# Ipuch/cocofest

Hardware: AMD Instinct MI355X
Metric: NLP callback evals/s (constraint+Jac) and wall-clock to Ipopt-equiv convergence (higher is better)
Workload: dtype f64; 1 GPU; cfg2: OcpFes DingModelFrequency n_stim=10 @10Hz, final_time=1s, n_shooting=20, end_node_tracking=100N, RK1 x 10 multiple shooting; one step = g + J_g of every instance; batch_per_gpu=1048576, nv=42, ng=40, nnz_jac=100, parallelism=instances sharded over 1 GPU(s), no data-path collective

## Files before the change

### cocofest_amd/csrc/cfx_chain.hip

```cpp
#include <hip/hip_runtime.h>

#include <algorithm>
#include <string>

#include "../../include/cfx.h"
#include "cfx_inertia.h"
#include "cfx_internal.h"

namespace cfx_chain {

typedef double d4 __attribute__((ext_vector_type(4)));

struct Chain {
    double *D, *L, *U;
    double *Cl, *Cr;
    int64_t stride, wstride;
    int M;
};

template <int SP>
__device__ __forceinline__ double* cur_u(const Chain& C, int64_t b, int k, int h) {
    constexpr int64_t NB = (int64_t)SP * SP;
    return h == 1 ? C.U + b * C.stride + k * NB : C.Cl + b * C.wstride + (k + h / 2) * NB;
}
template <int SP>
__device__ __forceinline__ double* cur_l(const Chain& C, int64_t b, int k, int h) {
    constexpr int64_t NB = (int64_t)SP * SP;
    return h == 1 ? C.L + b * C.stride + k * NB : C.Cr + b * C.wstride + (k - h / 2) * NB;
}

template <int SP, class AF>
__device__ __forceinline__ d4 tile_mm(const AF& a_at, const double (&breg)[SP / 4], int I, d4 acc) {
    const int lane = threadIdx.x & 63;
    const int r = 16 * I + (lane & 15), kq = lane >> 4;
#pragma unroll
    for (int kk = 0; kk < SP / 4; ++kk) acc = __builtin_amdgcn_mfma_f64_16x16x4f64(a_at(r, 4 * kk + kq), breg[kk], acc, 0, 0, 0);
    return acc;
}

template <int SP>
__device__ __forceinline__ void load_bcol(const double* __restrict__ B, int J, double (&breg)[SP / 4]) {
    const int lane = threadIdx.x & 63;
#pragma unroll
    for (int kk = 0; kk < SP / 4; ++kk) breg[kk] = B[(4 * kk + (lane >> 4)) * SP + 16 * J + (lane & 15)];
}

template <int SP>
__device__ __forceinline__ void store_tile(double* __restrict__ C, int I, int J, d4 v) {
    const int lane = threadIdx.x & 63;
#pragma unroll
    for (int r = 0; r < 4; ++r) C[(16 * I + (lane >> 4) + 4 * r) * SP + 16 * J + (lane & 15)] = v[r];
}

__device__ __forceinline__ double pivot_key(double v, int r) {
    const uint64_t bits = (uint64_t)__double_as_longlong(fabs(v));
    if (bits >= 0x7ff0000000000000ull) return -1.0;
    return __longlong_as_double((long long)((bits & ~0x7Full) | (uint64_t)(127 - r)));
}

#define CFX_DPP_MAX(v, CTRL, RM, BM)                                                                              \
    do {                                                                                                          \
        const int lo_ = __double2loint(v), hi_ = __double2hiint(v);                                               \
        const int slo_ = __builtin_amdgcn_update_dpp(lo_, lo_, CTRL, RM, BM, false);                              \
        const int shi_ = __builtin_amdgcn_update_dpp(hi_, hi_, CTRL, RM, BM, false);                              \
        v = fmax(v, __hiloint2double(shi_, slo_));                                                                \
    } while (0)
__device__ __forceinline__ double wave_max(double v) {
    CFX_DPP_MAX(v, 0x111, 0xf, 0xf);
    CFX_DPP_MAX(v, 0x112, 0xf, 0xf);
    CFX_DPP_MAX(v, 0x114, 0xf, 0xf);
    CFX_DPP_MAX(v, 0x118, 0xf, 0xf);
    CFX_DPP_MAX(v, 0x142, 0xa, 0xf);
    CFX_DPP_MAX(v, 0x143, 0xc, 0xf);
    const int lo = __builtin_amdgcn_readlane(__double2loint(v), 63), hi = __builtin_amdgcn_readlane(__double2hiint(v), 63);
    return __hiloint2double(hi, lo);
}

constexpr int kNT = 256;

__device__ __forceinline__ double readlane_d(double v, int l) {
    return __hiloint2double(__builtin_amdgcn_readlane(__double2hiint(v), l), __builtin_amdgcn_readlane(__double2loint(v), l));
}

template <int SP>
__global__ void __launch_bounds__(kNT) k_chain_elim(Chain C, int first, int step, int h, int32_t* __restrict__ info) {
    constexpr int T = SP / 16;
    static_assert(SP % 16 == 0 && SP <= 128 && kNT == 256, "16-column panels; 7-bit row index in the pivot key");
    constexpr int LDA = SP + 1;
    __shared__ double A[SP * LDA];
    __shared__ uint8_t prow[SP], pstep[SP];
    const int t = threadIdx.x, lane = t & 63, wave = t >> 6;
    const int i = first + step * blockIdx.x;
    const int64_t b = blockIdx.y;
    if (i >= C.M) return;
    constexpr int64_t NB = (int64_t)SP * SP;
    double* D = C.D + b * C.stride + i * NB;
    for (int e = t; e < SP * SP; e += kNT) A[(e / SP) * LDA + e % SP] = D[e];
    for (int r = t; r < SP; r += kNT) pstep[r] = 255;
    __syncthreads();
    int sing = 0;
    bool used0 = false, used1 = false;
    const bool has0 = lane < SP, has1 = lane + 64 < SP;
#pragma unroll 1
    for (int j = 0; j < T; ++j) {
        if (wave == 0) {
            double a0[16], a1[16];
#pragma unroll
            for (int c = 0; c < 16; ++c) {
                a0[c] = has0 ? A[lane * LDA + 16 * j + c] : 0.0;
                a1[c] = has1 ? A[(lane + 64) * LDA + 16 * j + c] : 0.0;
            }
#pragma unroll
            for (int kk = 0; kk < 16; ++kk) {
                const int k = 16 * j + kk;
                double key = -1.0;
                if (has0 && !used0) key = pivot_key(a0[kk], lane);
                if (has1 && !used1) key = fmax(key, pivot_key(a1[kk], lane + 64));
                key = wave_max(key);
                int p;
                if (key >= 0.0) {
                    p = 127 - (int)((uint64_t)__double_as_longlong(key) & 0x7Full);
                } else {
                    const unsigned long long m0 = __ballot(has0 && !used0), m1 = __ballot(has1 && !used1);
                    p = m0 ? __ffsll((long long)m0) - 1 : 64 + __ffsll((long long)m1) - 1;
                    if (!sing) sing = k + 1;
                }
                used0 = used0 || p == lane;
                used1 = used1 || p == lane + 64;
                if (lane == 0) prow[k] = (uint8_t)p, pstep[p] = (uint8_t)k;
                double prv[16];
                if (p < 64) {
#pragma unroll
                    for (int c = 0; c < 16; ++c) prv[c] = readlane_d(a0[c], p);
                } else {
#pragma unroll
                    for (int c = 0; c < 16; ++c) prv[c] = readlane_d(a1[c], p - 64);
                }
                const double pv = prv[kk];
                if (pv == 0.0 && !sing) sing = k + 1;
                const double inv = pv != 0.0 ? 1.0 / pv : 0.0;
                double sc[16];
#pragma unroll
                for (int c = 0; c < 16; ++c) sc[c] = c == kk ? inv : prv[c] * inv;
                const bool ip0 = lane == p, ip1 = lane + 64 == p;
                const double m0 = a0[kk], m1 = a1[kk];
#pragma unroll
                for (int c = 0; c < 16; ++c) {
                    if (c == kk) continue;
                    a0[c] = ip0 ? sc[c] : fma(-m0, sc[c], a0[c]);
                    a1[c] = ip1 ? sc[c] : fma(-m1, sc[c], a1[c]);
                }
                a0[kk] = ip0 ? inv : -m0 * inv;
                a1[kk] = ip1 ? inv : -m1 * inv;
            }
#pragma unroll
            for (int c = 0; c < 16; ++c) {
                if (has0) A[lane * LDA + 16 * j + c] = a0[c];
                if (has1) A[(lane + 64) * LDA + 16 * j + c] = a1[c];
            }
        }
        __syncthreads();
        for (int q = wave; q < T - 1; q += kNT / 64) {
            const int Jc = q < j ? q : q + 1;
            double breg[4];
#pragma unroll
            for (int kk = 0; kk < 4; ++kk) breg[kk] = A[prow[16 * j + 4 * kk + (lane >> 4)] * LDA + 16 * Jc + (lane & 15)];
#pragma unroll 1
            for (int I = 0; I < T; ++I) {
                d4 acc;
#pragma unroll
                for (int r = 0; r < 4; ++r) {
                    const int row = 16 * I + (lane >> 4) + 4 * r;
                    const int ps = pstep[row];
                    const bool piv = ps >= 16 * j && ps < 16 * j + 16;
                    acc[r] = piv ? 0.0 : A[row * LDA + 16 * Jc + (lane & 15)];
                }
#pragma unroll
                for (int kk = 0; kk < 4; ++kk)
                    acc = __builtin_amdgcn_mfma_f64_16x16x4f64(A[(16 * I + (lane & 15)) * LDA + 16 * j + 4 * kk + (lane >> 4)],
                                                               breg[kk], acc, 0, 0, 0);
#pragma unroll
                for (int r = 0; r < 4; ++r) A[(16 * I + (lane >> 4) + 4 * r) * LDA + 16 * Jc + (lane & 15)] = acc[r];
            }
        }
        __syncthreads();
    }
    const int tr = t >> 4, tc = t & 15;
    double a[T][T];
#pragma unroll
    for (int ii = 0; ii < T; ++ii)
#pragma unroll
        for (int jj = 0; jj < T; ++jj) a[ii][jj] = A[prow[tr + 16 * ii] * LDA + pstep[tc + 16 * jj]];
    __syncthreads();
#pragma unroll
    for (int ii = 0; ii < T; ++ii)
#pragma unroll
        for (int jj = 0; jj < T; ++jj) A[(tr + 16 * ii) * LDA + tc + 16 * jj] = a[ii][jj];
    __syncthreads();
    if (t == 0 && sing && info && info[b] == 0) info[b] = (int32_t)(i * SP + sing);
    for (int e = t; e < SP * SP; e += kNT) D[e] = A[(e / SP) * LDA + e % SP];
    auto a_at = [&](int r, int c) { return A[r * LDA + c]; };
    const bool xl = i - h >= 0, yu = i + h < C.M;
    for (int it = wave; it < 2 * (SP / 16); it += kNT / 64) {
        const int side = it / (SP / 16), J = it % (SP / 16);
        if (side == 0 ? !xl : !yu) continue;
        double* Bm = side == 0 ? cur_l<SP>(C, b, i, h) : cur_u<SP>(C, b, i, h);
        double breg[SP / 4];
        load_bcol<SP>(Bm, J, breg);
#pragma unroll 1
        for (int I = 0; I < SP / 16; ++I) {
            d4 acc = {0.0, 0.0, 0.0, 0.0};
            acc = tile_mm<SP>(a_at, breg, I, acc);
            store_tile<SP>(Bm, I, J, acc);
        }
    }
}

constexpr int kUpdGlobalB = 256;
template <int SP>
constexpr bool chain_b_fits() {
    return 2 * SP * (SP + 1) * 8 <= 150 * 1024;
}
template <int SP, bool BLDS>
constexpr size_t chain_upd_lds() {
    return (size_t)(BLDS ? 2 : 1) * SP * (SP + 1) * sizeof(double);
}
template <int SP, bool BLDS>
__global__ void __launch_bounds__(kNT) k_chain_upd(Chain C, int h) {
    constexpr int T16 = SP / 16, NT = T16 * T16, TPW = (NT + 3) / 4;
    constexpr int LD = SP + 1;
    constexpr bool BL = BLDS && chain_b_fits<SP>();
    extern __shared__ double sm[];
    double* sA = sm;
    double* sB = sm + SP * LD;
    const int t = threadIdx.x, wave = t >> 6, lane = t & 63;
    const int p = 2 * h * blockIdx.x, part = blockIdx.z;
    const int64_t b = blockIdx.y;
    if (p >= C.M) return;
    constexpr int64_t NB = (int64_t)SP * SP;
    const int i = p + h, j = p - h;
    const bool hi = i < C.M, hj = j >= 0;
    const bool hyi = hi && i + h < C.M;
    if ((part == 0 && !hi && !hj) || (part == 1 && !hi) || (part == 2 && !hj)) return;
    const double* Up = hi ? cur_u<SP>(C, b, p, h) : nullptr;
    const double* Lp = hj ? cur_l<SP>(C, b, p, h) : nullptr;
    d4 acc[TPW];
#pragma unroll
    for (int q = 0; q < TPW; ++q) acc[q] = d4{0.0, 0.0, 0.0, 0.0};
    auto product = [&](const double* __restrict__ Ag, const double* __restrict__ Bg) {
        __syncthreads();
        for (int e = t; e < SP * SP; e += kNT) {
            const int r = e / SP, c = e - r * SP;
            sA[r * LD + c] = Ag[e];
            if constexpr (BL) sB[r * LD + c] = Bg[e];
        }
        __syncthreads();
#pragma unroll
        for (int q = 0; q < TPW; ++q) {
            const int tile = wave + 4 * q;
            if (tile < NT) {
                const int I = tile / T16, J = tile % T16;
                const int ra = 16 * I + (lane & 15), kq = lane >> 4, cb = 16 * J + (lane & 15);
                d4 a = acc[q];
#pragma unroll
                for (int kk = 0; kk < SP / 4; ++kk) {
                    const double bv = BL ? sB[(4 * kk + kq) * LD + cb] : Bg[(4 * kk + kq) * SP + cb];
                    a = __builtin_amdgcn_mfma_f64_16x16x4f64(sA[ra * LD + 4 * kk + kq], bv, a, 0, 0, 0);
                }
                acc[q] = a;
            }
        }
    };
    double* out;
    if (part == 0) {
        if (hi) product(Up, cur_l<SP>(C, b, i, h));
        if (hj) product(Lp, cur_u<SP>(C, b, j, h));
        out = C.D + b * C.stride + p * NB;
    } else if (part == 1) {
        if (hyi) product(Up, cur_u<SP>(C, b, i, h));
        out = C.Cl + b * C.wstride + i * NB;
    } else {
        product(Lp, cur_l<SP>(C, b, j, h));
        out = C.Cr + b * C.wstride + j * NB;
    }
#pragma unroll
    for (int q = 0; q < TPW; ++q) {
        const int tile = wave + 4 * q;
        if (tile < NT) {
            const int I = tile / T16, J = tile % T16;
#pragma unroll
            for (int r = 0; r < 4; ++r) {
                const int64_t e = (16 * I + (lane >> 4) + 4 * r) * SP + 16 * J + (lane & 15);
                if (part == 0) out[e] -= acc[q][r];
                else out[e] = -acc[q][r];
            }
        }
    }
}

template <int SP>
__device__ __forceinline__ double row_dot(const double* __restrict__ Mx, int r, const double* x) {
    double a0 = 0.0, a1 = 0.0, a2 = 0.0, a3 = 0.0;
    const double* row = Mx + (int64_t)r * SP;
#pragma unroll 4
    for (int k = 0; k < SP; k += 4) {
        a0 = fma(row[k], x[k], a0);
        a1 = fma(row[k + 1], x[k + 1], a1);
        a2 = fma(row[k + 2], x[k + 2], a2);
        a3 = fma(row[k + 3], x[k + 3], a3);
    }
    return (a0 + a1) + (a2 + a3);
}

struct Rhs {
    double* R;
    int64_t r_inst, r_rhs;
    double* T;
    int64_t t_inst, t_rhs;
};

template <int SP>
__global__ void __launch_bounds__(kNT) k_chain_fwd(Chain C, Rhs X, int h) {
    static_assert(SP <= 128, "rows over two thread halves");
    __shared__ double vi[SP], vj[SP], ti[SP], tj[SP];
    const int t = threadIdx.x;
    const int p = 2 * h * blockIdx.x;
    const int64_t b = blockIdx.z, c = blockIdx.y;
    if (p >= C.M) return;
    constexpr int64_t NB = (int64_t)SP * SP;
    const int i = p + h, j = p - h;
    const bool hi = i < C.M, hj = j >= 0;
    double* R = X.R + b * X.r_inst + c * X.r_rhs;
    double* T = X.T + b * X.t_inst + c * X.t_rhs;
    for (int r = t; r < SP; r += kNT) {
        vi[r] = hi ? R[(int64_t)i * SP + r] : 0.0;
        vj[r] = hj ? R[(int64_t)j * SP + r] : 0.0;
    }
    __syncthreads();
    if (t < SP) {
        if (hi) {
            const double v = row_dot<SP>(C.D + b * C.stride + i * NB, t, vi);
            ti[t] = v;
            T[(int64_t)i * SP + t] = v;
        }
    } else if (t >= 128 && t < 128 + SP) {
        if (hj) tj[t - 128] = row_dot<SP>(C.D + b * C.stride + j * NB, t - 128, vj);
    }
    __syncthreads();
    if (t < SP) {
        if (hi) vi[t] = row_dot<SP>(cur_u<SP>(C, b, p, h), t, ti);
    } else if (t >= 128 && t < 128 + SP) {
        if (hj) vj[t - 128] = row_dot<SP>(cur_l<SP>(C, b, p, h), t - 128, tj);
    }
    __syncthreads();
    if (t < SP && (hi || hj)) {
        double acc = R[(int64_t)p * SP + t];
        if (hi) acc -= vi[t];
        if (hj) acc -= vj[t];
        R[(int64_t)p * SP + t] = acc;
    }
}

template <int SP>
__global__ void __launch_bounds__(kNT) k_chain_top(Chain C, Rhs X) {
    __shared__ double v[SP];
    const int t = threadIdx.x;
    const int64_t b = blockIdx.z, c = blockIdx.y;
    double* R = X.R + b * X.r_inst + c * X.r_rhs;
    for (int r = t; r < SP; r += kNT) v[r] = R[r];
    __syncthreads();
    if (t < SP) R[t] = row_dot<SP>(C.D + b * C.stride, t, v);
}

template <int SP>
__global__ void __launch_bounds__(kNT) k_chain_bwd(Chain C, Rhs X, int h) {
    __shared__ double xl[SP], xr[SP];
    const int t = threadIdx.x;
    const int i = h + 2 * h * blockIdx.x;
    const int64_t b = blockIdx.z, c = blockIdx.y;
    if (i >= C.M) return;
    const bool hr = i + h < C.M;
    double* R = X.R + b * X.r_inst + c * X.r_rhs;
    const double* T = X.T + b * X.t_inst + c * X.t_rhs;
    for (int r = t; r < SP; r += kNT) {
        xl[r] = R[(int64_t)(i - h) * SP + r];
        xr[r] = hr ? R[(int64_t)(i + h) * SP + r] : 0.0;
    }
    __syncthreads();
    __shared__ double yl[SP], yr[SP];
    if (t < SP) yl[t] = row_dot<SP>(cur_l<SP>(C, b, i, h), t, xl);
    else if (t >= 128 && t < 128 + SP && hr) yr[t - 128] = row_dot<SP>(cur_u<SP>(C, b, i, h), t - 128, xr);
    __syncthreads();
    if (t < SP) {
        double acc = T[(int64_t)i * SP + t] - yl[t];
        if (hr) acc -= yr[t];
        R[(int64_t)i * SP + t] = acc;
    }
}

static int levels(int M) {
    int L = 0;
    while ((1 << L) < M) ++L;
    return L;
}

template <int SP, bool BL>
static hipError_t allow_upd_lds() {
    if (chain_upd_lds<SP, BL>() <= 65536) return hipSuccess;
    static const hipError_t e = hipFuncSetAttribute(reinterpret_cast<const void*>(&k_chain_upd<SP, BL>),
                                                    hipFuncAttributeMaxDynamicSharedMemorySize,
                                                    (int)chain_upd_lds<SP, BL>());
    return e;
}

template <int SP>
static hipError_t factor_sp(const Chain& C, int64_t B, int32_t* info, hipStream_t s) {
    const int L = levels(C.M);
    constexpr bool FITS = chain_b_fits<SP>();
    hipError_t e = allow_upd_lds<SP, FITS>();
    if (e == hipSuccess) e = allow_upd_lds<SP, false>();
    if (e != hipSuccess) return e;
    for (int l = 0; l < L; ++l) {
        const int h = 1 << l;
        const int ne = (C.M - h + 2 * h - 1) / (2 * h), ns = (C.M + 2 * h - 1) / (2 * h);
        hipLaunchKernelGGL(k_chain_elim<SP>, dim3((unsigned)ne, (unsigned)B), dim3(kNT), 0, s, C, h, 2 * h, h, info);
        if (FITS && ns < kUpdGlobalB)
            k_chain_upd<SP, FITS><<<dim3((unsigned)ns, (unsigned)B, 3), dim3(kNT), chain_upd_lds<SP, FITS>(), s>>>(C, h);
        else
            k_chain_upd<SP, false><<<dim3((unsigned)ns, (unsigned)B, 3), dim3(kNT), chain_upd_lds<SP, false>(), s>>>(C, h);
    }
    hipLaunchKernelGGL(k_chain_elim<SP>, dim3(1, (unsigned)B), dim3(kNT), 0, s, C, 0, 1, 1 << L, info);
    return hipGetLastError();
}

template <int SP>
static hipError_t solve_sp(const Chain& C, int64_t B, const Rhs& X, int nrhs, hipStream_t s) {
    const int L = levels(C.M);
    for (int l = 0; l < L; ++l) {
        const int h = 1 << l;
        const int ns = (C.M + 2 * h - 1) / (2 * h);
        hipLaunchKernelGGL(k_chain_fwd<SP>, dim3((unsigned)ns, (unsigned)nrhs, (unsigned)B), dim3(kNT), 0, s, C, X, h);
    }
    hipLaunchKernelGGL(k_chain_top<SP>, dim3(1, (unsigned)nrhs, (unsigned)B), dim3(kNT), 0, s, C, X);
    for (int l = L - 1; l >= 0; --l) {
        const int h = 1 << l;
        const int ne = (C.M - h + 2 * h - 1) / (2 * h);
        hipLaunchKernelGGL(k_chain_bwd<SP>, dim3((unsigned)ne, (unsigned)nrhs, (unsigned)B), dim3(kNT), 0, s, C, X, h);
    }
    return hipGetLastError();
}

template <int SP>
constexpr size_t chain_inertia_lds() {
    return (size_t)SP * (SP + 1) * sizeof(double);
}
template <int SP>
__global__ void __launch_bounds__(kNT) k_chain_inertia(Chain C, int32_t* __restrict__ neg) {
    extern __shared__ double A[];
    constexpr int64_t NB = (int64_t)SP * SP;
    const int64_t b = blockIdx.y;
    const double* D = C.D + b * C.stride + blockIdx.x * NB;
    for (int e = threadIdx.x; e < SP * SP; e += kNT) {
        const int r = e / SP, c = e % SP;
        A[r * (SP + 1) + c] = 0.5 * (D[r * SP + c] + D[c * SP + r]);
    }
    __syncthreads();
    const int cnt = cfx_inertia::sym_neg_count(A, SP + 1, SP);
    if (threadIdx.x == 0 && cnt) atomicAdd(neg + b, cnt);
}

template <int SP>
static hipError_t inertia_sp(const Chain& C, int64_t B, int32_t* neg, hipStream_t s) {
    if (chain_inertia_lds<SP>() > 65536) {
        static const hipError_t e = hipFuncSetAttribute(reinterpret_cast<const void*>(&k_chain_inertia<SP>),
                                                        hipFuncAttributeMaxDynamicSharedMemorySize,
                                                        (int)chain_inertia_lds<SP>());
        if (e != hipSuccess) return e;
    }
    k_chain_inertia<SP><<<dim3((unsigned)C.M, (unsigned)B), dim3(kNT), chain_inertia_lds<SP>(), s>>>(C, neg);
    return hipGetLastError();
}

#define CFX_CHAIN_SP(F, ...)                                     \
    switch (sp) {                                                \
        case 16: e = F<16>(__VA_ARGS__); break;                  \
        case 32: e = F<32>(__VA_ARGS__); break;                  \
        case 48: e = F<48>(__VA_ARGS__); break;                  \
        case 64: e = F<64>(__VA_ARGS__); break;                  \
        case 80: e = F<80>(__VA_ARGS__); break;                  \
        case 96: e = F<96>(__VA_ARGS__); break;                  \
        case 112: e = F<112>(__VA_ARGS__); break;                \
        case 128: e = F<128>(__VA_ARGS__); break;                \
        default: e = hipErrorInvalidValue; break;                \
    }

}

int cfx_chain_sp_ok(int32_t sp) { return sp >= 16 && sp <= 128 && sp % 16 == 0; }

int cfx_chain_factor_s(int64_t batch, int32_t M, int32_t sp, double* D, double* L, double* U, int64_t stride,
                       double* Cl, double* Cr, int64_t wstride, int32_t* info, void* stream) {
    if (batch < 1 || batch > 65535 || M < 1 || !cfx_chain_sp_ok(sp) || !D || !L || !U || !Cl || !Cr) {
        g_create_error = "cfx_chain_factor: invalid argument";
        return CFX_EINVAL;
    }
    const hipStream_t s = (hipStream_t)stream;
    if (info && hipMemsetAsync(info, 0, batch * sizeof(int32_t), s) != hipSuccess) {
        g_create_error = "cfx_chain_factor: hipMemsetAsync failed";
        return CFX_EHIP;
    }
    const cfx_chain::Chain C{D, L, U, Cl, Cr, stride, wstride, M};
    hipError_t e;
    CFX_CHAIN_SP(cfx_chain::factor_sp, C, batch, info, s)
    if (e != hipSuccess) {
        g_create_error = std::string("cfx_chain_factor: ") + hipGetErrorString(e);
        return CFX_EHIP;
    }
    return CFX_OK;
}

int cfx_chain_solve_s(int64_t batch, int32_t M, int32_t sp, const double* D, const double* L, const double* U,
                      int64_t stride, const double* Cl, const double* Cr, int64_t wstride, int32_t nrhs, double* R,
                      int64_t r_inst, int64_t r_rhs, double* T, int64_t t_inst, int64_t t_rhs, void* stream) {
    if (batch < 1 || batch > 65535 || M < 1 || !cfx_chain_sp_ok(sp) || nrhs < 1 || nrhs > 65535 || !R || !T) {
        g_create_error = "cfx_chain_solve: invalid argument";
        return CFX_EINVAL;
    }
    const cfx_chain::Chain C{const_cast<double*>(D), const_cast<double*>(L), const_cast<double*>(U),
                             const_cast<double*>(Cl), const_cast<double*>(Cr), stride, wstride, M};
    const cfx_chain::Rhs X{R, r_inst, r_rhs, T, t_inst, t_rhs};
    hipError_t e;
    CFX_CHAIN_SP(cfx_chain::solve_sp, C, batch, X, nrhs, (hipStream_t)stream)
    if (e != hipSuccess) {
        g_create_error = std::string("cfx_chain_solve: ") + hipGetErrorString(e);
        return CFX_EHIP;
    }
    return CFX_OK;
}

int cfx_chain_inertia_s(int64_t batch, int32_t M, int32_t sp, const double* D, int64_t stride, int32_t* neg,
                        void* stream) {
    if (batch < 1 || batch > 65535 || M < 1 || !cfx_chain_sp_ok(sp) || !D || !neg) {
        g_create_error = "cfx_chain_inertia: invalid argument";
        return CFX_EINVAL;
    }
    const cfx_chain::Chain C{const_cast<double*>(D), nullptr, nullptr, nullptr, nullptr, stride, 0, M};
    hipError_t e;
    CFX_CHAIN_SP(cfx_chain::inertia_sp, C, batch, neg, (hipStream_t)stream)
    if (e != hipSuccess) {
        g_create_error = std::string("cfx_chain_inertia: ") + hipGetErrorString(e);
        return CFX_EHIP;
    }
    return CFX_OK;
}

extern "C" int cfx_btri_factor(int64_t batch, int32_t M, int32_t sp, double* D, double* L, double* U, double* work,
                               int32_t* info, void* stream) {
    if (!work) {
        g_create_error = "cfx_btri_factor: work is NULL";
        return CFX_EINVAL;
    }
    const int64_t st = (int64_t)M * sp * sp;
    return cfx_chain_factor_s(batch, M, sp, D, L, U, st, work, work + batch * st, st, info, stream);
}

extern "C" int cfx_btri_solve(int64_t batch, int32_t M, int32_t sp, const double* D, const double* L, const double* U,
                              const double* work, int32_t nrhs, double* rhs, double* scratch, void* stream) {
    if (!work) {
        g_create_error = "cfx_btri_solve: work is NULL";
        return CFX_EINVAL;
    }
    const int64_t st = (int64_t)M * sp * sp, nv = (int64_t)M * sp;
    return cfx_chain_solve_s(batch, M, sp, D, L, U, st, work, work + batch * st, st, nrhs, rhs, nrhs * nv, nv, scratch,
                             nrhs * nv, nv, stream);
}

extern "C" int cfx_btri_inertia(int64_t batch, int32_t M, int32_t sp, const double* D, int32_t* neg, void* stream) {
    if (!neg || batch < 1 || batch > 65535) {
        g_create_error = "cfx_btri_inertia: invalid argument";
        return CFX_EINVAL;
    }
    if (hipMemsetAsync(neg, 0, batch * sizeof(int32_t), (hipStream_t)stream) != hipSuccess) {
        g_create_error = "cfx_btri_inertia: hipMemsetAsync failed";
        return CFX_EHIP;
    }
    return cfx_chain_inertia_s(batch, M, sp, D, (int64_t)M * sp * sp, neg, stream);
}
```

Baseline: 4.091 billion instance-evals/s.

## Stage chain-solve block matvecs through LDS panels with batched right-hand sides

```diff
diff --git a/cocofest_amd/csrc/cfx_chain.hip b/cocofest_amd/csrc/cfx_chain.hip
--- a/cocofest_amd/csrc/cfx_chain.hip
+++ b/cocofest_amd/csrc/cfx_chain.hip
@@ -1,6 +1,7 @@
 #include <hip/hip_runtime.h>
 
 #include <algorithm>
+#include <cstdlib>
 #include <string>
 
 #include "../../include/cfx.h"
@@ -398,6 +399,227 @@
     }
 }
 
+typedef double d2 __attribute__((ext_vector_type(2)));
+constexpr int kRG = 4;
+constexpr int kVPT = (kRG * 128 + kNT - 1) / kNT;
+
+template <int SP, int PW>
+struct Mv {
+    static_assert(SP % PW == 0 && PW % 8 == 0 && kNT == 256, "16-byte chunks, row stride = 4 mod 8");
+    static constexpr int LDP = PW + 4;
+    static constexpr int CPR = PW / 2;
+    static constexpr int NCH = 2 * SP * CPR;
+    static constexpr int NLD = (NCH + kNT - 1) / kNT;
+    static constexpr int NPAN = SP / PW;
+    static constexpr int NQ = 8 * SP;
+    static constexpr int NPQ = (NQ + kNT - 1) / kNT;
+    static constexpr int PANEL = 2 * SP * LDP;
+    static_assert((SP * CPR) % 64 == 0 && (4 * SP) % 64 == 0, "sides and tails are wave-uniform");
+    static constexpr size_t lds(int nr) { return (size_t)(PANEL + 4 * nr * SP) * sizeof(double); }
+};
+
+template <int SP, int PW>
+__device__ __forceinline__ void mv_load(const double* __restrict__ A0, const double* __restrict__ A1, int pan,
+                                        d2 (&reg)[Mv<SP, PW>::NLD]) {
+    using V = Mv<SP, PW>;
+#pragma unroll
+    for (int m = 0; m < V::NLD; ++m) {
+        const int e = threadIdx.x + m * kNT;
+        if (V::NCH % kNT != 0 && e >= V::NCH) continue;
+        const int side = e / (SP * V::CPR), rem = e - side * (SP * V::CPR), r = rem / V::CPR, cc = rem - r * V::CPR;
+        const double* __restrict__ A = side ? A1 : A0;
+        if (A) reg[m] = *reinterpret_cast<const d2*>(A + r * SP + pan * PW + 2 * cc);
+    }
+}
+
+template <int SP, int PW>
+__device__ __forceinline__ void mv_store(const d2 (&reg)[Mv<SP, PW>::NLD], double* sP) {
+    using V = Mv<SP, PW>;
+#pragma unroll
+    for (int m = 0; m < V::NLD; ++m) {
+        const int e = threadIdx.x + m * kNT;
+        if (V::NCH % kNT != 0 && e >= V::NCH) continue;
+        const int row = e / V::CPR, cc = e - row * V::CPR;
+        *reinterpret_cast<d2*>(sP + row * V::LDP + 2 * cc) = reg[m];
+    }
+}
+
+template <int SP, int PW, class Fill>
+__device__ __forceinline__ void mv_run(const double* __restrict__ A0, const double* __restrict__ A1,
+                                       const double* __restrict__ B0, const double* __restrict__ B1, int nph, double* sm,
+                                       int nr, double* Tout, int64_t t_rhs, const Fill& fill) {
+    using V = Mv<SP, PW>;
+    double* sP = sm;
+    double* va = sm + V::PANEL;
+    double* vb = va + 2 * nr * SP;
+    const int t = threadIdx.x;
+    d2 reg[V::NLD];
+    double acc[V::NPQ][kRG];
+#pragma unroll
+    for (int m = 0; m < V::NLD; ++m) reg[m] = d2{0.0, 0.0};
+#pragma unroll
+    for (int m = 0; m < V::NPQ; ++m)
+#pragma unroll
+        for (int c = 0; c < kRG; ++c) acc[m][c] = 0.0;
+    mv_load<SP, PW>(A0, A1, 0, reg);
+    fill();
+    const int nst = nph * V::NPAN;
+#pragma unroll 1
+    for (int s = 0; s < nst; ++s) {
+        const int ph = s / V::NPAN, pan = s - ph * V::NPAN;
+        __syncthreads();
+        mv_store<SP, PW>(reg, sP);
+        __syncthreads();
+        if (s + 1 < nst) {
+            const int ph1 = (s + 1) / V::NPAN, pan1 = s + 1 - ph1 * V::NPAN;
+            mv_load<SP, PW>(ph1 ? B0 : A0, ph1 ? B1 : A1, pan1, reg);
+        }
+        const bool h0 = (ph ? B0 : A0) != nullptr, h1 = (ph ? B1 : A1) != nullptr;
+        const double* x = ph ? vb : va;
+#pragma unroll
+        for (int m = 0; m < V::NPQ; ++m) {
+            const int q = t + m * kNT;
+            if (V::NQ % kNT != 0 && q >= V::NQ) continue;
+            const int side = q / (4 * SP), r = (q - side * 4 * SP) >> 2, j = q & 3;
+            if (!(side ? h1 : h0)) continue;
+            const double* row = sP + (side * SP + r) * V::LDP + j;
+#pragma unroll
+            for (int c = 0; c < kRG; ++c) {
+                if (c >= nr) break;
+                const double* xc = x + (side * nr + c) * SP + pan * PW + j;
+                double a = acc[m][c];
+#pragma unroll
+                for (int kk = 0; kk < PW / 4; ++kk) a = fma(row[4 * kk], xc[4 * kk], a);
+                acc[m][c] = a;
+            }
+        }
+        if (pan == V::NPAN - 1) {
+            double* y = ph ? va : vb;
+#pragma unroll
+            for (int m = 0; m < V::NPQ; ++m) {
+                const int q = t + m * kNT;
+                if (V::NQ % kNT != 0 && q >= V::NQ) continue;
+                const int side = q / (4 * SP), r = (q - side * 4 * SP) >> 2, j = q & 3;
+                if (!(side ? h1 : h0)) continue;
+#pragma unroll
+                for (int c = 0; c < kRG; ++c) {
+                    if (c >= nr) break;
+                    double v = acc[m][c];
+                    v = v + __shfl_xor(v, 1);
+                    v = v + __shfl_xor(v, 2);
+                    if (j == 0) {
+                        y[(side * nr + c) * SP + r] = v;
+                        if (ph == 0 && side == 0 && Tout) Tout[c * t_rhs + r] = v;
+                    }
+                    acc[m][c] = 0.0;
+                }
+            }
+        }
+    }
+    __syncthreads();
+}
+
+template <int SP, int PW>
+__device__ __forceinline__ void fwd_step(const Chain& C, const Rhs& X, int64_t b, int c0, int nr, int p, int h,
+                                         double* sm) {
+    constexpr int64_t NB = (int64_t)SP * SP;
+    const int t = threadIdx.x;
+    const int i = p + h, j = p - h;
+    const bool hi = i < C.M, hj = j >= 0;
+    double* R = X.R + b * X.r_inst + c0 * X.r_rhs;
+    double* T = X.T + b * X.t_inst + c0 * X.t_rhs;
+    double* va = sm + Mv<SP, PW>::PANEL;
+    double rp[kVPT];
+    mv_run<SP, PW>(hi ? C.D + b * C.stride + i * NB : nullptr, hj ? C.D + b * C.stride + j * NB : nullptr,
+                   hi ? cur_u<SP>(C, b, p, h) : nullptr, hj ? cur_l<SP>(C, b, p, h) : nullptr, 2, sm, nr,
+                   hi ? T + (int64_t)i * SP : nullptr, X.t_rhs, [&] {
+                       for (int e = t; e < 2 * nr * SP; e += kNT) {
+                           const int side = e / (nr * SP), rem = e - side * nr * SP, c = rem / SP, r = rem - c * SP;
+                           const bool ok = side ? hj : hi;
+                           va[e] = ok ? R[c * X.r_rhs + (int64_t)(side ? j : i) * SP + r] : 0.0;
+                       }
+#pragma unroll
+                       for (int m = 0; m < kVPT; ++m) {
+                           const int e = t + m * kNT, c = e / SP, r = e - c * SP;
+                           rp[m] = e < nr * SP ? R[c * X.r_rhs + (int64_t)p * SP + r] : 0.0;
+                       }
+                   });
+    if (!hi && !hj) return;
+#pragma unroll
+    for (int m = 0; m < kVPT; ++m) {
+        const int e = t + m * kNT, c = e / SP, r = e - c * SP;
+        if (e >= nr * SP) break;
+        double acc = rp[m];
+        if (hi) acc -= va[e];
+        if (hj) acc -= va[nr * SP + e];
+        R[c * X.r_rhs + (int64_t)p * SP + r] = acc;
+    }
+}
+
+template <int SP, int PW>
+__device__ __forceinline__ void top_step(const Chain& C, const Rhs& X, int64_t b, int c0, int nr, double* sm) {
+    const int t = threadIdx.x;
+    double* R = X.R + b * X.r_inst + c0 * X.r_rhs;
+    double* va = sm + Mv<SP, PW>::PANEL;
+    double* vb = va + 2 * nr * SP;
+    mv_run<SP, PW>(C.D + b * C.stride, nullptr, nullptr, nullptr, 1, sm, nr, nullptr, 0, [&] {
+        for (int e = t; e < nr * SP; e += kNT) va[e] = R[(e / SP) * X.r_rhs + e % SP];
+    });
+    for (int e = t; e < nr * SP; e += kNT) R[(e / SP) * X.r_rhs + e % SP] = vb[e];
+}
+
+template <int SP, int PW>
+__device__ __forceinline__ void bwd_step(const Chain& C, const Rhs& X, int64_t b, int c0, int nr, int i, int h,
+                                         double* sm) {
+    const int t = threadIdx.x;
+    const bool hr = i + h < C.M;
+    double* R = X.R + b * X.r_inst + c0 * X.r_rhs;
+    const double* T = X.T + b * X.t_inst + c0 * X.t_rhs;
+    double* va = sm + Mv<SP, PW>::PANEL;
+    double* vb = va + 2 * nr * SP;
+    double ti[kVPT];
+    mv_run<SP, PW>(cur_l<SP>(C, b, i, h), hr ? cur_u<SP>(C, b, i, h) : nullptr, nullptr, nullptr, 1, sm, nr, nullptr, 0,
+                   [&] {
+        for (int e = t; e < 2 * nr * SP; e += kNT) {
+            const int side = e / (nr * SP), rem = e - side * nr * SP, c = rem / SP, r = rem - c * SP;
+            va[e] = side && !hr ? 0.0 : R[c * X.r_rhs + (int64_t)(side ? i + h : i - h) * SP + r];
+        }
+#pragma unroll
+        for (int m = 0; m < kVPT; ++m) {
+            const int e = t + m * kNT, c = e / SP, r = e - c * SP;
+            ti[m] = e < nr * SP ? T[c * X.t_rhs + (int64_t)i * SP + r] : 0.0;
+        }
+    });
+#pragma unroll
+    for (int m = 0; m < kVPT; ++m) {
+        const int e = t + m * kNT, c = e / SP, r = e - c * SP;
+        if (e >= nr * SP) break;
+        double acc = ti[m] - vb[e];
+        if (hr) acc -= vb[nr * SP + e];
+        R[c * X.r_rhs + (int64_t)i * SP + r] = acc;
+    }
+}
+
+extern __shared__ __attribute__((aligned(16))) double chain_sm[];
+
+template <int SP, int PW>
+__global__ void __launch_bounds__(kNT) k_chain_fwd_st(Chain C, Rhs X, int h, int nrhs) {
+    const int p = 2 * h * blockIdx.x, c0 = kRG * blockIdx.y;
+    if (p >= C.M) return;
+    fwd_step<SP, PW>(C, X, blockIdx.z, c0, min(kRG, nrhs - c0), p, h, chain_sm);
+}
+template <int SP, int PW>
+__global__ void __launch_bounds__(kNT) k_chain_bwd_st(Chain C, Rhs X, int h, int nrhs) {
+    const int i = h + 2 * h * blockIdx.x, c0 = kRG * blockIdx.y;
+    if (i >= C.M) return;
+    bwd_step<SP, PW>(C, X, blockIdx.z, c0, min(kRG, nrhs - c0), i, h, chain_sm);
+}
+template <int SP, int PW>
+__global__ void __launch_bounds__(kNT) k_chain_top_st(Chain C, Rhs X, int nrhs) {
+    const int c0 = kRG * blockIdx.y;
+    top_step<SP, PW>(C, X, blockIdx.z, c0, min(kRG, nrhs - c0), chain_sm);
+}
+
 static int levels(int M) {
     int L = 0;
     while ((1 << L) < M) ++L;
@@ -434,7 +656,7 @@
 }
 
 template <int SP>
-static hipError_t solve_sp(const Chain& C, int64_t B, const Rhs& X, int nrhs, hipStream_t s) {
+static hipError_t solve_levels_sp(const Chain& C, int64_t B, const Rhs& X, int nrhs, hipStream_t s) {
     const int L = levels(C.M);
     for (int l = 0; l < L; ++l) {
         const int h = 1 << l;
@@ -446,6 +668,56 @@
         const int h = 1 << l;
         const int ne = (C.M - h + 2 * h - 1) / (2 * h);
         hipLaunchKernelGGL(k_chain_bwd<SP>, dim3((unsigned)ne, (unsigned)nrhs, (unsigned)B), dim3(kNT), 0, s, C, X, h);
+    }
+    return hipGetLastError();
+}
+
+inline bool chain_solve_levels() {
+    const char* e = std::getenv("CFX_CHAIN_SOLVE");
+    return e && std::string(e) == "levels";
+}
+constexpr int kWidePanels = 256;
+
+template <class K>
+static hipError_t allow_lds(K kernel, size_t bytes) {
+    if (bytes <= 65536) return hipSuccess;
+    return hipFuncSetAttribute(reinterpret_cast<const void*>(kernel), hipFuncAttributeMaxDynamicSharedMemorySize,
+                               (int)bytes);
+}
+
+template <int SP>
+static hipError_t solve_sp(const Chain& C, int64_t B, const Rhs& X, int nrhs, hipStream_t s) {
+    const uintptr_t bits = reinterpret_cast<uintptr_t>(C.D) | reinterpret_cast<uintptr_t>(C.L) |
+                           reinterpret_cast<uintptr_t>(C.U) | reinterpret_cast<uintptr_t>(C.Cl) |
+                           reinterpret_cast<uintptr_t>(C.Cr);
+    const bool aligned = (bits & 15) == 0 && (B == 1 || ((C.stride | C.wstride) & 1) == 0);
+    if (chain_solve_levels() || !aligned) return solve_levels_sp<SP>(C, B, X, nrhs, s);
+    constexpr int PN = SP <= 80 ? SP : SP / 2, PWD = 16;
+    static const hipError_t attr = [] {
+        hipError_t e = allow_lds(&k_chain_fwd_st<SP, PN>, Mv<SP, PN>::lds(kRG));
+        if (e == hipSuccess) e = allow_lds(&k_chain_bwd_st<SP, PN>, Mv<SP, PN>::lds(kRG));
+        if (e == hipSuccess) e = allow_lds(&k_chain_top_st<SP, PN>, Mv<SP, PN>::lds(kRG));
+        return e;
+    }();
+    if (attr != hipSuccess) return attr;
+    const int L = levels(C.M);
+    constexpr int wide = kWidePanels;
+    const int nr = std::min(nrhs, kRG), ng = (nrhs + kRG - 1) / kRG;
+    const size_t ldn = Mv<SP, PN>::lds(nr), ldw = Mv<SP, PWD>::lds(nr);
+    for (int l = 0; l < L; ++l) {
+        const int h = 1 << l;
+        const int ns = (C.M + 2 * h - 1) / (2 * h);
+        const dim3 g((unsigned)ns, (unsigned)ng, (unsigned)B);
+        if (ns * ng * B >= wide) k_chain_fwd_st<SP, PWD><<<g, dim3(kNT), ldw, s>>>(C, X, h, nrhs);
+        else k_chain_fwd_st<SP, PN><<<g, dim3(kNT), ldn, s>>>(C, X, h, nrhs);
+    }
+    k_chain_top_st<SP, PN><<<dim3(1, (unsigned)ng, (unsigned)B), dim3(kNT), ldn, s>>>(C, X, nrhs);
+    for (int l = L - 1; l >= 0; --l) {
+        const int h = 1 << l;
+        const int ne = (C.M - h + 2 * h - 1) / (2 * h);
+        const dim3 g((unsigned)ne, (unsigned)ng, (unsigned)B);
+        if (ne * ng * B >= wide) k_chain_bwd_st<SP, PWD><<<g, dim3(kNT), ldw, s>>>(C, X, h, nrhs);
+        else k_chain_bwd_st<SP, PN><<<g, dim3(kNT), ldn, s>>>(C, X, h, nrhs);
     }
     return hipGetLastError();
 }
```

Result: slower. 4.044 billion instance-evals/s (-1.1%).
